# reinforcement-learning-kr/alpha_omok

Measured on AMD Instinct MI355X. Metric: self-play move-decisions/sec (9x9, 400 sims/move), higher is better.
Workload: dtype f32 (fp16x2-split MFMA operands, 3 products per multiply-add, f32 accumulate; inter-layer activations stored as two fp16 halves: ~22 significand bits)

## Files before the change

### alpha_omok_amd/csrc/net.hip

```cpp
#include <hip/hip_runtime.h>

#include <cmath>
#include <cstdio>
#include <cstdlib>
#include <cstring>
#include <map>
#include <type_traits>
#include <string>
#include <thread>
#include <vector>

#include "../../include/omok_hip.h"
#include "engine_types.hpp"
#include "net_device.hpp"
#include "net_common.hpp"
#include "net_trunk_f32.hpp"
#include "net_trunk_h16.hpp"
#include "net_layer_ksplit.hpp"
#include "net_board_h16.hpp"
#include "net_small.hpp"
#include "net_w16.hpp"


struct ao_net {
    int nb = 0, C = 0, planes = 0, B = 0, A = 0, device = 0;
    int nchq32 = 0;
    int nchq16 = 0;
    int CQ = 0;
    int mode = 0;
    int requested_mode = 0;
    int fp16_fallbacks = 0;
    bool forced_fp32 = false;
    int num_cu = 256;
    bool finalized = false;
    std::string err;
    std::map<std::string, std::vector<float>> params;
    std::vector<void*> allocs;
    std::vector<std::pair<void*, size_t>> pallocs;
    size_t pcursor = 0;
    std::vector<float*> conv_w, conv_sc, conv_sh;
    std::vector<uint4*> convh_wh, convh_wl;
    uint4 *step_w1h = nullptr, *step_w1l = nullptr;
    std::vector<float*> convh_sc;
    float* conv0_w16 = nullptr;
    float* conv0_w1 = nullptr;
    int nchq1 = 0;
    float *head_w3 = nullptr, *head_sc3 = nullptr, *head_sh3 = nullptr;
    float *wp_t = nullptr, *bp = nullptr, *w1_t = nullptr, *b1 = nullptr, *w2 = nullptr, *b2 = nullptr;
    int ws_boards = 0;
    float *act_x = nullptr, *act_t = nullptr, *hbuf = nullptr, *il_in = nullptr;
    float *tmp_p = nullptr, *tmp_v = nullptr;
    int* d_status = nullptr;
    bool attr_l[16][2] = {}, attr_done[16] = {}, lds_attr_done[16] = {}, attr_k[16] = {};
    int ksplit_min = 48, ksplit_max = 64, ksplit_max2 = 0;
    int rowk_min = 1, rowk_max = 47;
    bool attr_r[16] = {};
    int boardk_min = 64;
    bool attr_b[16] = {};
    long perboard_cells = 2592;
    int force_xt = 0, force_nch = 0;
    bool timing = false;
    bool timing_on = false;
    int timing_stride = 1;
    unsigned timing_tick = 0;
    static constexpr int kRing = 512;
    std::vector<hipEvent_t> ev0, ev1;
    int ring_head = 0, ring_count = 0;
    double ms_total = 0.0;
    int64_t launches = 0;
    int last_in_kind = 1;
    bool w16 = false;
    int products_req = 0;
    int trunk_fmt = -1;

    int fail(const std::string& m) { err = m; return 1; }
};

#define NET_HIP(n, call)                                                                      \
    do {                                                                                      \
        hipError_t st_ = (call);                                                              \
        if (st_ != hipSuccess)                                                                \
            return (n)->fail(std::string(#call) + ": " + hipGetErrorString(st_));             \
    } while (0)

static thread_local std::string g_net_create_error;

template <typename T>
static int net_alloc(ao_net* n, T** out, size_t count) {
    void* p = nullptr;
    hipError_t st = hipMalloc(&p, std::max<size_t>(count * sizeof(T), 16));
    if (st != hipSuccess) return n->fail(std::string("hipMalloc: ") + hipGetErrorString(st));
    n->allocs.push_back(p);
    *out = static_cast<T*>(p);
    return 0;
}

template <typename T>
static int param_alloc(ao_net* n, T** out, size_t count) {
    const size_t bytes = std::max<size_t>(count * sizeof(T), 16);
    if (n->pcursor < n->pallocs.size() && n->pallocs[n->pcursor].second == bytes) {
        *out = static_cast<T*>(n->pallocs[n->pcursor++].first);
        return 0;
    }
    void* p = nullptr;
    hipError_t st = hipMalloc(&p, bytes);
    if (st != hipSuccess) return n->fail(std::string("hipMalloc: ") + hipGetErrorString(st));
    if (n->pcursor < n->pallocs.size()) {
        (void)hipFree(n->pallocs[n->pcursor].first);
        n->pallocs[n->pcursor] = {p, bytes};
    } else {
        n->pallocs.push_back({p, bytes});
    }
    ++n->pcursor;
// ... 243 lines not shown
            switch (n->B) {
#define AO_CELLS_LAUNCH2(W, Q, NWV)                                                                           \
    hipLaunchKernelGGL((k_conv_cells<W, Q, NWV>), grid, block, 0, s, reinterpret_cast<const float4*>(in), w4, \
                       reinterpret_cast<const float4*>(n->conv_sc[layer]),                                   \
                       reinterpret_cast<const float4*>(n->conv_sh[layer]), reinterpret_cast<const float4*>(res), \
                       reinterpret_cast<float4*>(out), cqi, n->planes, res ? 1 : 0)
#define AO_CELLS_LAUNCH(W, Q)                                                                                 \
    do {                                                                                                      \
        if (nw == 9) AO_CELLS_LAUNCH2(W, Q, 9);                                                               \
        else AO_CELLS_LAUNCH2(W, Q, 3);                                                                       \
    } while (0)
#define AO_BW_CASE(W)                                                                                         \
    case W:                                                                                                   \
        switch (cqi >> 2) {                                                                                   \
            case 1: AO_CELLS_LAUNCH(W, 1); break;                                                             \
            case 2: AO_CELLS_LAUNCH(W, 2); break;                                                             \
            case 4: AO_CELLS_LAUNCH(W, 4); break;                                                             \
            case 6: AO_CELLS_LAUNCH(W, 6); break;                                                             \
            default: AO_CELLS_LAUNCH(W, 8); break;                                                            \
        }                                                                                                     \
        break;
                AO_BW_CASE(3) AO_BW_CASE(4) AO_BW_CASE(5) AO_BW_CASE(6) AO_BW_CASE(7) AO_BW_CASE(8) AO_BW_CASE(9)
                AO_BW_CASE(10) AO_BW_CASE(11) AO_BW_CASE(12) AO_BW_CASE(13) AO_BW_CASE(14) AO_BW_CASE(15)
#undef AO_BW_CASE
#undef AO_CELLS_LAUNCH
#undef AO_CELLS_LAUNCH2
            }
            if (timed) timer_end(n, idx, s);
        };
        if (parts & 1) conv(0, in_il, n->nchq1, nullptr, n->act_x);
        for (int i = 0; i < n->nb && (parts & 2); ++i) {
            conv(1 + 2 * i, n->act_x, n->CQ, nullptr, n->act_t);
            conv(2 + 2 * i, n->act_t, n->CQ, n->act_x, n->act_x);
        }
        const size_t lds1 = heads_lds_floats(n->A, n->planes) * sizeof(float);
        if (parts & 4)
            hipLaunchKernelGGL(k_heads_board, dim3(boards), dim3(1024), lds1, s, head_params(n),
                               reinterpret_cast<const float4*>(n->act_x), policy, value, n->A, n->planes);
        NET_HIP(n, hipGetLastError());
#ifdef AO_PROF
        if (getenv("AO_PROF_PRINT")) {
            unsigned long long h[8];
            hipStreamSynchronize(s);
            hipMemcpyFromSymbol(h, HIP_SYMBOL(ao_prof_heads), sizeof(h));
            unsigned long long cv[8];
            hipMemcpyFromSymbol(cv, HIP_SYMBOL(ao_prof_conv), sizeof(cv));
            fprintf(stderr, "AO_PROF k_conv_cells_h (last layer, block 0, wave 0) ticks: rows loaded + split + stored %llu, barrier + LDS reads + MFMAs %llu, reduction barrier %llu, reduce+epilogue+store %llu, total %llu\n",
                    cv[1] - cv[0], cv[2] - cv[1], cv[3] - cv[2], cv[4] - cv[3], cv[4] - cv[0]);
            fprintf(stderr, "AO_PROF k_heads_board ticks: w3 %llu, 1x1 conv %llu, reduce %llu, FC %llu, softmax+value %llu, tanh/store %llu, total %llu\n",
                    h[1] - h[0], h[2] - h[1], h[3] - h[2], h[4] - h[3], h[5] - h[4], h[6] - h[5], h[6] - h[0]);
        }
#endif
        return 0;
#ifdef AO_PROF
    } else if (group == 16 && mode == 5 && (layers_only(n) || !(n->B <= 9 && (groups >= 192 || getenv("AO_FORCE_RESIDENT"))))) {
#else
    } else if (group == 16 && mode == 5 && (layers_only(n) || !(n->B <= 9 && groups >= 192))) {
#endif
        int xt = n->B, nchh = 1;
        {
            double best = -1.0;
            const int xts[2] = {5, 4};
            for (int k = 0; k < (n->B <= 9 ? 1 : 2); ++k) {
                const int x = n->B <= 9 ? n->B : xts[k];
                const int ntile = (n->B + x - 1) / x;
                const int staged_cols = n->B <= 9 ? x : x + 2;
                for (int c = 1; c <= n->B; ++c) {
                    const long rounds = (static_cast<long>(groups) * c * ntile + n->num_cu - 1) / n->num_cu;
                    const int rows = (n->B + c - 1) / c;
                    const int staged_rows = rows + (c > 1 ? 2 : 0);
                    const double cost = rounds * (static_cast<double>(rows) * x + 0.25 * staged_rows * staged_cols + 2.0);
                    if (best < 0 || cost < best) { best = cost; nchh = c; xt = x; }
                }
            }
            if (n->force_xt > 0 && n->B > 9) xt = n->force_xt;
            if (n->force_nch > 0) nchh = n->force_nch;
        }
        const int nxt = (n->B + xt - 1) / xt;
        const int ks = (!layers_only(n) && n->B >= 4 && n->B <= 9 && groups >= n->ksplit_min) ? (groups <= n->ksplit_max ? 4 : groups <= n->ksplit_max2 ? 2 : 0) : 0;
        const bool rowk = !layers_only(n) && n->B >= 4 && n->B <= 9 && groups >= n->rowk_min && groups <= n->rowk_max;
        const bool ksplit = ks != 0 || rowk;
        auto layer_k = [&](int l) -> int {
            LayerHArgs a;
            a.src = static_cast<const void*>((l & 1) ? n->act_x : n->act_t);
            a.dst = reinterpret_cast<uint4*>(!(l & 1) ? n->act_x : n->act_t);
            a.layer.wh = n->convh_wh[l];
            a.layer.wl = n->convh_wl[l];
            a.layer.sc = reinterpret_cast<const float4*>(n->convh_sc[l]);
            a.layer.sh = reinterpret_cast<const float4*>(n->conv_sh[l]);
            a.layer.ovf = n->d_status;
            a.res = !(l & 1) ? 1 : 0;
            a.nch = groups;
            a.live = live; a.row_cap = row_cap;
            const dim3 grid(rowk ? (groups + 7) / 8 * 8 * 4 * n->B : (groups + 7) / 8 * 8 * ks), block(512);
            const int idx = n->timing ? timer_begin(n, s) : 0;
            if (two_products(n) && (rowk || ks == 4)) {
                if (rowk) NET_HIP(n, ao::launch_row16hk_w16(n->device, n->B, grid, s, a));
                else NET_HIP(n, ao::launch_layer16hk_w16(n->device, n->B, grid, s, a));
                if (n->timing) timer_end(n, idx, s);
                return 0;
            }
            if (rowk) {
                switch (n->B) {
#define AO_BW_CASE(W)                                                                                                  \
    case W: {                                                                                                          \
        constexpr size_t lds_ = static_cast<size_t>(W) * 8 * 1024;                                                     \
        if (!n->attr_r[W]) {                                                                                           \
            NET_HIP(n, hipFuncSetAttribute(reinterpret_cast<const void*>(&k_row16hk<W>),                               \
                                           hipFuncAttributeMaxDynamicSharedMemorySize, static_cast<int>(lds_)));       \
            n->attr_r[W] = true;                                                                                       \
        }                                                                                                              \
// ... 290 lines not shown
namespace ao {
void net_fp16_fallback_begin(ao_net* n) {
    ++n->fp16_fallbacks;
    n->mode = 2;
}
int net_fp16_fallback_end(ao_net* n) {
    n->forced_fp32 = n->fp16_fallbacks >= 3;
    if (!n->forced_fp32) n->mode = n->requested_mode;
    return n->forced_fp32 ? 1 : 0;
}
}

extern "C" {

const char* ao_net_last_error(const ao_net* n) { return n ? n->err.c_str() : g_net_create_error.c_str(); }

int ao_net_create(int n_block, int inplanes, int planes, int board, int device, ao_net** out) {
    if (!out) return 1;
    *out = nullptr;
    auto bad = [&](const char* m) { g_net_create_error = m; return 1; };
    if (n_block < 0 || n_block > 64) return bad("n_block out of range");
    if (inplanes < 1 || inplanes > 12) return bad("inplanes must be in 1..12");
    if (planes < 32 || planes > 512 || planes % 32) return bad("planes must be a multiple of 32 in 32 .. 512");
    if (board < 3 || board > ao::kMaxBoard) return bad("board must be in 3..15");
    int ndev = 0;
    if (hipGetDeviceCount(&ndev) != hipSuccess || ndev <= 0) return bad("no HIP device available");
    if (device < 0 || device >= ndev) return bad("device ordinal out of range");
    ao_net* n = new ao_net();
    n->nb = n_block; n->C = inplanes; n->planes = planes; n->B = board; n->A = board * board;
    n->device = device;
    n->nchq32 = (((inplanes + 3) / 4) + 1) & ~1;
    n->nchq16 = (((inplanes + 3) / 4) + 7) & ~7;
    n->nchq1 = (((inplanes + 3) / 4) + 3) & ~3;
    n->CQ = planes / 4;
    {
        hipDeviceProp_t prop;
        if (hipGetDeviceProperties(&prop, device) == hipSuccess && prop.multiProcessorCount > 0)
            n->num_cu = prop.multiProcessorCount;
    }
    if (const char* v = getenv("AO_KSPLIT")) {
        int lo = 0, hi = 0, hi2 = 0;
        if (sscanf(v, "%d,%d,%d", &lo, &hi, &hi2) == 3) { n->ksplit_min = lo > 0 ? lo : 1 << 30; n->ksplit_max = hi; n->ksplit_max2 = hi2; }
    }
    if (const char* v = getenv("AO_PERBOARD_CELLS")) n->perboard_cells = atol(v);
    if (const char* v = getenv("AO_BOARDK")) n->boardk_min = atoi(v);
    if (const char* v = getenv("AO_ROWK")) {
        int lo = 0, hi = -1;
        if (sscanf(v, "%d,%d", &lo, &hi) == 2) { n->rowk_min = lo; n->rowk_max = hi; }
    }
    if (const char* v = getenv("AO_TRUNK_FMT")) n->trunk_fmt = atoi(v) == 1 ? 1 : 0;
    if (n->trunk_fmt < 0) n->trunk_fmt = 0;
    if (const char* v = getenv("AO_XT")) n->force_xt = atoi(v) == 4 ? 4 : (atoi(v) == 5 ? 5 : 0);
    if (const char* v = getenv("AO_NCH")) n->force_nch = atoi(v) > 0 && atoi(v) <= board ? atoi(v) : 0;
    *out = n;
    return 0;
}

void ao_net_destroy(ao_net* n) {
    if (!n) return;
    hipSetDevice(n->device);
    hipDeviceSynchronize();
    for (void* p : n->allocs) hipFree(p);
    for (auto& pa : n->pallocs) hipFree(pa.first);
    for (auto e : n->ev0) hipEventDestroy(e);
    for (auto e : n->ev1) hipEventDestroy(e);
    delete n;
}

int ao_net_set_mode(ao_net* n, int mode) {
    if (mode < 0 || mode > 6)
        return n->fail("mode must be 0 (auto), 1 (layer kernels), 2 (group-resident trunk), 3 (per-board), 4 (row-chunked), 5 (split-fp16 trunk) "
                       "or 6 (split-fp16 per-layer kernels for every batch size)");
    if ((mode == 5 || mode == 6) && !h16_supported(n))
        return n->fail("modes 5 / 6 (split-fp16 MFMA trunk) need 128 planes and at least one ResBlock");
    n->mode = n->requested_mode = mode;
    n->forced_fp32 = false;
    return 0;
}


int ao_net_get_mode(const ao_net* n) { return n->mode; }

int ao_net_set_param(ao_net* n, const char* name, const float* data, int64_t numel) {
    if (!name || (!data && numel > 0) || numel < 0) return n->fail("bad argument");
    n->params[name] = std::vector<float>(data, data + numel);
    n->finalized = false;
    return 0;
}

static int get_param(ao_net* n, const std::string& name, size_t numel, const std::vector<float>** out) {
    auto it = n->params.find(name);
    if (it == n->params.end()) return n->fail("missing parameter " + name);
    if (it->second.size() != numel)
        return n->fail("parameter " + name + " has " + std::to_string(it->second.size()) + " elements, expected " +
                       std::to_string(numel));
    *out = &it->second;
    return 0;
}

static int fold_bn(ao_net* n, const std::string& prefix, int c, std::vector<float>* sc, std::vector<float>* sh) {
    const std::vector<float>*w, *b, *m, *v;
    if (get_param(n, prefix + ".weight", c, &w) || get_param(n, prefix + ".bias", c, &b) ||
        get_param(n, prefix + ".running_mean", c, &m) || get_param(n, prefix + ".running_var", c, &v))
        return 1;
    sc->resize(c); sh->resize(c);
    for (int i = 0; i < c; ++i) {
// ... 213 lines not shown
    NET_HIP(n, hipSetDevice(n->device));
    hipStream_t s = static_cast<hipStream_t>(stream);
    int32_t f = 0;
    NET_HIP(n, hipMemcpyAsync(&f, n->d_status, sizeof(int32_t), hipMemcpyDeviceToHost, s));
    NET_HIP(n, hipStreamSynchronize(s));
    if (clear && f) {
        NET_HIP(n, hipMemsetAsync(n->d_status, 0, sizeof(int32_t), s));
        NET_HIP(n, hipStreamSynchronize(s));
    }
    if (flags) *flags = f;
    return 0;
}

int ao_net_conv_timing(ao_net* n, int enable, double* ms_total, int64_t* launches) {
    NET_HIP(n, hipSetDevice(n->device));
    if (n->ev0.empty() && enable) {
        n->ev0.resize(ao_net::kRing);
        n->ev1.resize(ao_net::kRing);
        for (int i = 0; i < ao_net::kRing; ++i) {
            NET_HIP(n, hipEventCreate(&n->ev0[i]));
            NET_HIP(n, hipEventCreate(&n->ev1[i]));
        }
    }
    harvest(n, n->ring_count);
    if (ms_total) *ms_total = n->ms_total;
    if (launches) *launches = n->launches;
    n->ms_total = 0.0;
    n->launches = 0;
    n->timing_on = enable != 0;
    n->timing_stride = enable > 1 ? enable : 1;
    n->timing_tick = 0;
    n->timing = false;
    return 0;
}

static void dominant_name(const ao_net* n, int boards, int in_kind, std::string* nm_out, double* f_out) {
    int group = 32, nchq = 0;
    ao::net_plan(n, boards, &group, &nchq, nullptr);
    const int padded = (boards + group - 1) / group * group;
    const double conv = 2.0 * n->A * 9.0 * n->planes * n->planes * padded;
    const double conv1 = 2.0 * n->A * 9.0 * n->C * n->planes * padded;
    const int mode = ao::pick_mode_public(n, boards);
    const std::string bw = std::to_string(n->B);
    std::string nm;
    double f;
    if (group == 1) {
        nm = h16_supported(n) ? std::string(two_products(n) ? "k_conv_cells_h_w16<" : "k_conv_cells_h<") + bw + ", 8> (one 3x3 conv, per-board NHWC, board rows in LDS, split-fp16 MFMA 16x16x32, " +
                                    (two_products(n) ? "2 products: the conv weights are fp16 numbers)" : "3 products)")
                              : "k_conv_cells<" + bw + "> (one 3x3 conv, per-board NHWC, fp32 MFMA 16x16x4)";
        f = conv;
    } else if (group == 16 && mode == 4) {
        nm = "k_layer16<" + bw + "> (one 3x3 conv per launch, 16-board groups x row chunks, fp32 MFMA 16x16x4)";
        f = conv;
    } else if (group == 16 && mode == 5 && !layers_only(n) && n->B >= 4 && n->B <= 9 && (boards + 15) / 16 >= n->rowk_min &&
               (boards + 15) / 16 <= n->rowk_max) {
        nm = std::string(two_products(n) ? "k_row16hk_w16<" : "k_row16hk<") + bw + "> (one 3x3 conv per launch as split-fp16 MFMA 16x16x32 (" +
             (two_products(n) ? "2 products: the conv weights are fp16 numbers" : "3 products") + ", fp32 accumulate): one workgroup per "
             "16-board group x output row x cout pair, waves split the contraction by input block, partial tiles exchanged through LDS)";
        f = conv;
    } else if (group == 16 && mode == 5 && !layers_only(n) && n->B >= 4 && n->B <= 9 && (boards + 15) / 16 >= n->ksplit_min &&
               (boards + 15) / 16 <= std::max(n->ksplit_max, n->ksplit_max2)) {
        const bool four = (boards + 15) / 16 <= n->ksplit_max;
        const bool two = two_products(n) && four;
        nm = std::string(two ? "k_layer16hk_w16<" : "k_layer16hk<") + bw + (four ? ", 4" : ", 2") + "> (one 3x3 conv per launch as split-fp16 MFMA 16x16x32 (" +
             (two ? "2 products: the conv weights are fp16 numbers" : "3 products") + ", fp32 accumulate): "
             "a 16-board group split over " + (four ? "four workgroups by cout pairs" : "two workgroups by cout quads") +
             ", waves split the contraction by input block, partial tiles exchanged through LDS)";
        f = conv;
    } else if (group == 16 && mode == 5 && board_resident(n, boards)) {
        nm = std::string(two_products(n) ? "k_boardh_w16<" : "k_boardh<") + bw + (in_kind == 2 ? ", 2" : ", 1") + "> (" + (in_kind == 2 ? "conv1 + " : "") + std::to_string(2 * n->nb) +
             " 3x3 convs in one launch as split-fp16 MFMA 16x16x32 (" + (two_products(n) ? "2 products: the conv weights are fp16 numbers" : "3 products") + ", fp32 accumulate): "
             "a workgroup = one board resident in LDS through all layers, the row's cells as the MFMA N dimension, column shifts as DPP row shifts)";
        f = 2.0 * n->nb * 2.0 * n->A * 9.0 * n->planes * n->planes * boards + (in_kind == 2 ? 2.0 * n->A * 9.0 * n->C * n->planes * boards : 0.0);
    } else if (group == 16 && mode == 5 && (layers_only(n) || !(n->B <= 9 && (boards + 15) / 16 >= 192))) {
        nm = std::string(two_products(n) ? "k_layer16h_w16<" : "k_layer16h<") + bw + "> (one 3x3 conv per launch as split-fp16 MFMA 16x16x32 (" +
             (two_products(n) ? "2 products: the conv weights are fp16 numbers" : "3 products") + ", fp32 accumulate), "
             "16-board groups x row chunks x column tiles)";
        f = conv;
    } else if (group == 16 && mode == 5) {
        const bool two = two_products(n) && n->trunk_fmt != 1;
        nm = std::string(in_kind == 2 ? "k_trunk16hb" : "k_trunk16h") + (two ? "_w16<" : "<") + bw + ", 4, " + std::to_string(n->trunk_fmt) + "> (conv1 + " +
             std::to_string(2 * n->nb) + " 3x3 convs as split-fp16 MFMA 16x16x32 (" + (two ? "2 products: the conv weights are fp16 numbers" : "3 products") + ", fp32 accumulate) + heads, one resident "
             "launch; activations between layers as " + (n->trunk_fmt == 1 ? "fp16 high half + one low byte" : "two fp16 halves") + ")";
        f = conv1 + 2.0 * n->nb * conv;
    } else if (group == 16) {
        nm = "k_trunk16<" + bw + "> (conv1 + " + std::to_string(2 * n->nb) + " 3x3 convs, one launch, fp32 MFMA 16x16x4)";
        f = conv1 + 2.0 * n->nb * conv;
    } else {
        nm = "k_conv3x3<" + bw + "> (one 3x3 " + std::to_string(n->planes) + "->" + std::to_string(n->planes) +
             " conv, fp32 MFMA 32x32x2)";
        f = conv;
    }
    *nm_out = nm;
    *f_out = f;
}

static void copy_name(const std::string& nm, char* name, int name_cap) {
    if (name && name_cap > 0) {
        std::strncpy(name, nm.c_str(), static_cast<size_t>(name_cap) - 1);
        name[name_cap - 1] = 0;
    }
}

int ao_net_products(ao_net* n, int32_t request, int32_t* in_force, int32_t* weights_fp16) {
    if (request != -1 && request != 0 && request != 3) return n->fail("ao_net_products: request must be -1 (query), 0 (automatic) or 3");
    if (request != -1) n->products_req = request;
    if (in_force) *in_force = two_products(n) ? 2 : 3;
    if (weights_fp16) *weights_fp16 = n->w16 ? 1 : 0;
    return 0;
}

int ao_net_dominant_kernel(ao_net* n, int boards, char* name, int name_cap, double* flop_per_launch) {
    std::string nm;
    double f = 0.0;
    dominant_name(n, boards, n->last_in_kind, &nm, &f);
    copy_name(nm, name, name_cap);
    if (flop_per_launch) *flop_per_launch = f;
    return 0;
}

int ao_net_plan_kernel(int n_block, int inplanes, int planes, int board, int trunk_mode, int boards, int in_kind,
                       char* name, int name_cap, double* flop_per_launch) {
    if (n_block < 0 || inplanes < 1 || planes < 32 || planes % 32 || board < 3 || board > ao::kMaxBoard || boards < 1 ||
        trunk_mode < 0 || trunk_mode > 6)
        return 1;
    ao_net n;
    n.nb = n_block; n.C = inplanes; n.planes = planes; n.B = board; n.A = board * board;
// ... 17 lines not shown
```

### alpha_omok_amd/csrc/net_trunk_h16.hpp

```cpp
#pragma once

namespace ao {

struct TrunkHLayer {
    const uint4* wh;
    const uint4* wl;
    const float4* sc;
    const float4* sh;
    int* ovf;
};

struct TrunkHArgs {
    const float4* in0;
    uint4* bufA;
    uint4* bufB;
    int nlayers;
    int CQ, COUT;
    const float *w3, *sc3, *sh3, *wp_t, *bp, *w1_t, *b1, *w2, *b2;
    float* policy;
    float* value;
    const unsigned* live;
    unsigned row_cap;
    TrunkHLayer layers[kMaxTrunkLayers];
};

typedef unsigned int u32x2 __attribute__((ext_vector_type(2)));
__device__ __forceinline__ half8 buf_ld_h8(__amdgpu_buffer_rsrc_t r, int voff, int soff) {
    return __builtin_bit_cast(half8, __builtin_amdgcn_raw_buffer_load_b128(r, voff, soff, 0));
}
#ifndef AO_AUX_RES
#define AO_AUX_RES 0
#endif
#ifndef AO_AUX_ST
#define AO_AUX_ST 0
#endif
#ifndef AO_AUX_STAGE
#define AO_AUX_STAGE 0
#endif
__device__ __forceinline__ half4 buf_ld_h4(__amdgpu_buffer_rsrc_t r, int voff, int soff) {
    return __builtin_bit_cast(half4, __builtin_amdgcn_raw_buffer_load_b64(r, voff, soff, AO_AUX_RES));
}
__device__ __forceinline__ void buf_st_h4(half4 v, __amdgpu_buffer_rsrc_t r, int voff, int soff) {
    __builtin_amdgcn_raw_buffer_store_b64(__builtin_bit_cast(u32x2, v), r, voff, soff, AO_AUX_ST);
}

#ifdef AO_PROF
static __device__ unsigned long long ao_prof[8 * 12];
#define AO_T(x) const unsigned long long x = __builtin_amdgcn_s_memtime()
#define AO_ACC(k, t0, t1) prof[k] += (t1) - (t0)
#else
#define AO_T(x)
#define AO_ACC(k, t0, t1)
#endif
// ... 9 lines not shown
}
__device__ __forceinline__ uint4 ao_ko_fragment(unsigned seed, bool low) {
    unsigned wd[4];
#pragma unroll
    for (int k = 0; k < 4; ++k) {
        unsigned out = 0;
#pragma unroll
        for (int h = 0; h < 2; ++h) {
            const unsigned r = ao_ko_hash(seed * 8u + k * 2u + h);
            const unsigned e = (low ? 4u : 15u) - ((r >> 10) & 7u);
            const unsigned v = (r & 0x80000000u) ? 0u : ((e << 10) | (r & 0x3ffu));
            out |= v << (16 * h);
        }
        wd[k] = out;
    }
    return make_uint4(wd[0], wd[1], wd[2], wd[3]);
}
#if AO_KO != 0 && !defined(AO_PROF) && !defined(AO_WRONG_RESULTS_OK)
#error "AO_KO builds compute wrong results on purpose: timing only, build them with -DAO_PROF"
#endif
#ifndef AO_SPLIT_BARRIER
#define AO_SPLIT_BARRIER 0
#endif
#ifndef AO_CONV1_SPLIT
#define AO_CONV1_SPLIT 0
#endif
__device__ __forceinline__ void row_arrive(unsigned* cnt, int lane) {
    asm volatile("s_waitcnt vmcnt(0) lgkmcnt(0)" ::: "memory");
    if (lane == 0) __hip_atomic_fetch_add(cnt, 1u, __ATOMIC_RELAXED, __HIP_MEMORY_SCOPE_WORKGROUP);
}
__device__ __forceinline__ void row_wait(unsigned* cnt, unsigned target) {
    for (;;) {
        const unsigned v = __hip_atomic_load(cnt, __ATOMIC_RELAXED, __HIP_MEMORY_SCOPE_WORKGROUP);
        if (__builtin_amdgcn_readfirstlane(v) >= target) break;
        __builtin_amdgcn_s_sleep(1);
    }
    asm volatile("" ::: "memory");
}

__host__ __device__ constexpr int kPlaneRow(int bw) { return bw * bw <= 128 ? 128 : 256; }
__host__ __device__ constexpr unsigned kPairBytes(int fmt) { return fmt == 1 ? 1536u : 2048u; }

constexpr float kLo8Scale = 0x1p-112f;
__device__ __forceinline__ float lo8_scaled(unsigned h, unsigned l) { return __uint_as_float(((h << 8) | l) << 5); }
__device__ __forceinline__ unsigned lo8_word(float vs) {
    const unsigned u = __float_as_uint(vs);
    return (u + 15u + ((u >> 5) & 1u)) >> 5;
}

template <int BW, int NC32, int NCI, int KIND, int FMT = 0, bool W16 = false>
struct TrunkHLayerFn {
static __device__ __forceinline__ void run(const void* src, uint4* dst, const TrunkHLayer& L, const bool RES, uint4* s_x,
                                           int tile, int lane, unsigned long long* prof, const bool flip,
                                           unsigned* s_cnt, const unsigned rows_before) {
    constexpr bool FIRST = KIND != 0;
    constexpr bool BITS = KIND == 2;
    auto py = [&](int y) { return flip ? BW - 1 - y : y; };
    constexpr int A = BW * BW;
    constexpr int NT = NC32 * 2;
    constexpr int NSP = 2;
    constexpr int NFR = BW * NCI * NSP;
    constexpr int NB = NCI * 3;
    constexpr int NPR = 3;
    constexpr int PAIR = static_cast<int>(kPairBytes(FMT));
    constexpr int NPAIR = BW * NCI;
    const int kq = lane >> 4, b = lane & 15;
    const int lane16 = lane * 16;
    const int out_voff = (((tile & 1) * 2 + (kq >> 1)) * 16 + b) * 16 + (kq & 1) * 8;
    float4 sc = L.sc[tile * 4 + kq], sh = L.sh[tile * 4 + kq];
    if (FMT == 1) {
        sc.x *= kLo8Scale; sc.y *= kLo8Scale; sc.z *= kLo8Scale; sc.w *= kLo8Scale;
        sh.x *= kLo8Scale; sh.y *= kLo8Scale; sh.z *= kLo8Scale; sh.w *= kLo8Scale;
    }
    const __amdgpu_buffer_rsrc_t rs_wh = make_rsrc(L.wh, 9u * NCI * NT * 1024u);
    const __amdgpu_buffer_rsrc_t rs_wl = make_rsrc(L.wl, 9u * NCI * NT * 1024u);
    const __amdgpu_buffer_rsrc_t rs_src =
        make_rsrc(src, BITS ? 16u * kPlaneRow(BW) : FIRST ? static_cast<unsigned>(A) * 8u * 16u * 16u : static_cast<unsigned>(A) * NCI * kPairBytes(FMT));
    const __amdgpu_buffer_rsrc_t rs_dst = make_rsrc(dst, static_cast<unsigned>(A) * NC32 * kPairBytes(FMT));
    half8 wA[2][3], wB[2][3], wres[2][FIRST ? 9 : 1];
    auto load_w = [&](int slab, half8 (&W)[2][3]) {
        if (FIRST) return;
        if (AO_KO == 1 && slab > 2) return;
        const int c = (slab / 3) % NCI, dy = slab % 3;
#pragma unroll
        for (int dx = 0; dx < 3; ++dx) {
            const int ub = ((((flip ? 2 - dy : dy) * 3 + dx) * NCI + c) * NT + tile) * 1024;
            W[0][dx] = buf_ld_h8(rs_wh, lane16, ub);
            if (!W16) W[1][dx] = buf_ld_h8(rs_wl, lane16, ub);
        }
    };
    if (FIRST) {
#pragma unroll
        for (int t = 0; t < 9; ++t) {
            wres[0][t] = buf_ld_h8(rs_wh, lane16, (t * NT + tile) * 1024);
            if (!W16) wres[1][t] = buf_ld_h8(rs_wl, lane16, (t * NT + tile) * 1024);
        }
    }
    auto load_planes = [&](int cell, int split) -> half8 {
        if (BITS) {
            const unsigned bits = __builtin_amdgcn_raw_buffer_load_b8(rs_src, b * kPlaneRow(BW) + cell, 0, 0);
            half8 h;
#pragma unroll
            for (int k = 0; k < 8; ++k)
                h[k] = (kq == 0 && split == 0 && ((bits >> k) & 1u)) ? static_cast<_Float16>(1.0f) : static_cast<_Float16>(0.0f);
            return h;
        }
        const int o = ((cell * 8 + 2 * kq) * 16 + b) * 16;
        const u32x4 q0 = __builtin_amdgcn_raw_buffer_load_b128(rs_src, o, 0, 0);
        const u32x4 q1 = __builtin_amdgcn_raw_buffer_load_b128(rs_src, o + 256, 0, 0);
        half8 h;
#pragma unroll
        for (int k = 0; k < 4; ++k) {
            const float v0 = __uint_as_float(q0[k]), v1 = __uint_as_float(q1[k]);
            const _Float16 h0 = static_cast<_Float16>(v0), h1 = static_cast<_Float16>(v1);
            h[k] = split ? static_cast<_Float16>(v0 - static_cast<float>(h0)) : h0;
            h[4 + k] = split ? static_cast<_Float16>(v1 - static_cast<float>(h1)) : h1;
        }
        return h;
    };
    float peak = 0.f;
    unsigned pbits[BITS ? (NFR + NT - 1) / NT : 1] = {};
    f32x4 acc[3][BW];
#pragma unroll
    for (int r = 0; r < 3; ++r)
#pragma unroll
        for (int i = 0; i < BW; ++i) acc[r][i] = f32x4{0.f, 0.f, 0.f, 0.f};
    auto epilogue = [&](int yo) {
        constexpr int HB = (BW + 1) / 2;
#pragma unroll
        for (int i0 = 0; i0 < BW; i0 += HB) {
            half4 rh[HB], rl[HB];
            unsigned rb[HB];
            if (RES) {
#pragma unroll
                for (int k = 0; k < HB; ++k) {
                    const int i = i0 + k < BW ? i0 + k : BW - 1;
                    const int ob = ((py(yo) * BW + i) * NC32 + (tile >> 1)) * PAIR;
                    rh[k] = buf_ld_h4(rs_dst, out_voff, ob);
                    if (FMT == 1) {
                        rb[k] = __builtin_amdgcn_raw_buffer_load_b32(rs_dst, out_voff >> 1, ob + 1024, AO_AUX_RES);
                    } else if (AO_KO == 10 || AO_KO == 12) {
                        const unsigned u = __builtin_amdgcn_raw_buffer_load_b32(rs_dst, out_voff >> 1, ob + 1024, AO_AUX_RES);
                        rl[k] = __builtin_bit_cast(half4, u32x2{u, u});
                    } else {
                        rl[k] = buf_ld_h4(rs_dst, out_voff, ob + 1024);
                    }
                }
            }
#pragma unroll
            for (int k = 0; k < HB; ++k) {
                const int i = i0 + k;
                if (i >= BW) continue;
                const f32x4 c = acc[0][i];
                float f[4] = {fmaf(c[0], sc.x, sh.x), fmaf(c[1], sc.y, sh.y), fmaf(c[2], sc.z, sh.z), fmaf(c[3], sc.w, sh.w)};
                const int ob = ((py(yo) * BW + i) * NC32 + (tile >> 1)) * PAIR;
                if (RES) {
                    if (FMT == 1) {
                        const u32x2 hb = __builtin_bit_cast(u32x2, rh[k]);
#pragma unroll
                        for (int r = 0; r < 4; ++r)
                            f[r] += lo8_scaled((hb[r >> 1] >> (16 * (r & 1))) & 0xffffu, (rb[k] >> (8 * r)) & 0xffu);
                    } else {
#pragma unroll
                        for (int r = 0; r < 4; ++r) f[r] += static_cast<float>(rh[k][r]) + static_cast<float>(rl[k][r]);
                    }
                }
                peak = fmaxf(fmaxf(peak, fmaxf(f[0], f[1])), fmaxf(f[2], f[3]));
                if (FMT == 1) {
                    unsigned t[4];
#pragma unroll
                    for (int r = 0; r < 4; ++r)
                        t[r] = lo8_word(f[r] >= 0x1p-126f ? fminf(f[r], 65504.f * kLo8Scale) : 0.f);
                    const u32x2 hw = {(t[0] >> 8) | ((t[1] >> 8) << 16), (t[2] >> 8) | ((t[3] >> 8) << 16)};
                    const unsigned lw = (t[0] & 0xffu) | ((t[1] & 0xffu) << 8) | ((t[2] & 0xffu) << 16) | (t[3] << 24);
                    __builtin_amdgcn_raw_buffer_store_b64(hw, rs_dst, out_voff, ob, AO_AUX_ST);
                    __builtin_amdgcn_raw_buffer_store_b32(lw, rs_dst, out_voff >> 1, ob + 1024, AO_AUX_ST);
                    continue;
                }
                half4 hh, hl;
#pragma unroll
                for (int r = 0; r < 4; ++r) {
                    const float v = fminf(fmaxf(f[r], 0.f), 65504.f);
                    hh[r] = static_cast<_Float16>(v);
                    hl[r] = static_cast<_Float16>(v - static_cast<float>(hh[r]));
                }
                buf_st_h4(hh, rs_dst, out_voff, ob);
                if (AO_KO == 10 || AO_KO == 12) __builtin_amdgcn_raw_buffer_store_b32(__builtin_bit_cast(u32x2, hl)[0], rs_dst, out_voff >> 1, ob + 1024, AO_AUX_ST);
                else
                buf_st_h4(hl, rs_dst, out_voff, ob + 1024);
            }
        }
    };
    auto stage_pairs = [&](int y, uint4* xb, int k0, int k1) {
#pragma unroll
        for (int k = k0; k < k1; ++k) {
            const int p = tile + NT * k;
            if (p < NPAIR) {
                const int so = (py(y) * NPAIR + p) * PAIR;
                __builtin_amdgcn_raw_ptr_buffer_load_lds(rs_src, (__attribute__((address_space(3))) void*)(xb + (2 * p) * 64), 16, lane16,
                                                         so, 0, AO_AUX_STAGE);
                if (lane < 32)
                    __builtin_amdgcn_raw_ptr_buffer_load_lds(rs_src, (__attribute__((address_space(3))) void*)(xb + (2 * p + 1) * 64), 16,
                                                             lane16, so + 1024, 0, AO_AUX_STAGE);
            }
        }
    };
    auto expand_pairs = [&](uint4* xb, int k0, int k1) {
        typedef _Float16 half2v __attribute__((ext_vector_type(2)));
        const half2v k18 = {static_cast<_Float16>(0x1p-18f), static_cast<_Float16>(0x1p-18f)};
        const half2v m8 = {static_cast<_Float16>(-0x1p-8f), static_cast<_Float16>(-0x1p-8f)};
#pragma unroll
        for (int k = k0; k < k1; ++k) {
            const int p = tile + NT * k;
            if (p < NPAIR) {
                const uint4 hv = xb[(2 * p) * 64 + lane];
                const u32x2 lv = reinterpret_cast<const u32x2*>(xb + (2 * p + 1) * 64)[lane];
                const unsigned hw[4] = {hv.x, hv.y, hv.z, hv.w};
                unsigned ow[4];
#pragma unroll
                for (int j = 0; j < 4; ++j) {
                    const unsigned y = __builtin_amdgcn_perm(0x64646464u, lv[j >> 1], (j & 1) ? 0x04030402u : 0x04010400u);
                    const half2v c = __builtin_elementwise_fma(__builtin_bit_cast(half2v, y), k18, m8);
                    const half2v sc2 = __builtin_bit_cast(half2v, hw[j] & 0x7c007c00u);
                    ow[j] = __builtin_bit_cast(unsigned, c * sc2);
                }
                xb[(2 * p + 1) * 64 + lane] = make_uint4(ow[0], ow[1], ow[2], ow[3]);
            }
        }
    };

    AO_T(t_a);
    __syncthreads();
    AO_T(t_a1);
    if (FIRST) {
#pragma unroll
        for (int k = 0; k < (NFR + NT - 1) / NT; ++k) {
            const int f = tile + NT * k;
            if (f < NFR) s_x[f * 64 + lane] = __builtin_bit_cast(uint4, load_planes(f >> 1, f & 1));
        }
    } else if (FMT == 1) {
        stage_pairs(0, s_x, 0, (NPAIR + NT - 1) / NT);
    } else if (!(AO_KO == 13 || AO_KO == 15)) {
#pragma unroll
        for (int k = 0; k < (NFR + NT - 1) / NT; ++k) {
            const int f = tile + NT * k;
            if (f < NFR && !(AO_KO == 10 && (f & 1) && lane >= 32))
                __builtin_amdgcn_raw_ptr_buffer_load_lds(rs_src, (__attribute__((address_space(3))) void*)(s_x + f * 64), 16,
                                                         (AO_KO == 12 && (f & 1) && lane >= 32) ? lane16 - 512 : lane16,
                                                         (py(0) * NFR + f) * 1024, 0, AO_AUX_STAGE);
        }
    }
    AO_T(t_a2);
    load_w(0, wA);
    asm volatile("s_waitcnt vmcnt(0) lgkmcnt(0)" ::: "memory");
    if (FMT == 1 && !FIRST) {
        expand_pairs(s_x, 0, (NPAIR + NT - 1) / NT);
        asm volatile("s_waitcnt lgkmcnt(0)" ::: "memory");
    }
    AO_T(t_a3);
    __syncthreads();
    AO_T(t_b);
    AO_ACC(0, t_a, t_b);
    AO_ACC(8, t_a, t_a1);
    AO_ACC(9, t_a1, t_a2);
    AO_ACC(10, t_a2, t_a3);
    AO_ACC(11, t_a3, t_b);

    for (int yi = 0; yi < BW; ++yi) {
        AO_T(t_r0);
        const uint4* xs = s_x + static_cast<size_t>(yi & 1) * NFR * 64;
        uint4* xn = s_x + static_cast<size_t>((yi + 1) & 1) * NFR * 64;
        const int yn = yi + 1 < BW ? yi + 1 : yi;
#pragma unroll
        for (int slab = 0; slab < NB; ++slab) {
            const int c = slab / 3, dy = slab % 3;
            half8 (&w)[2][3] = (slab & 1) ? wB : wA;
            half8 (&wn)[2][3] = (slab & 1) ? wA : wB;
            load_w(slab + 1, wn);
            if (dy == 1 && !AO_KO_NOSTAGE && FMT == 1 && !FIRST) {
                constexpr int K2 = (NPAIR / NT + NCI - 1) / (NCI > 1 ? NCI - 1 : 1);
                if (c > 0 && AO_KO != 11) expand_pairs(xn, (c - 1) * K2, c * K2);
                if (c + 1 < NCI) stage_pairs(yn, xn, c * K2, (c + 1) * K2);
            } else if (BITS && !AO_KO_NOSTAGE && AO_CONV1_SPLIT) {
                constexpr int KF = (NFR + NT - 1) / NT;
#pragma unroll
                for (int k = 0; k < KF; ++k) {
                    const int f = tile + NT * k;
                    if (f < NFR) {
                        if (dy == 0 && !(f & 1))
                            pbits[k] = __builtin_amdgcn_raw_buffer_load_b8(rs_src, b * kPlaneRow(BW) + yn * BW + (f >> 1), 0, 0);
                        if (dy == 2) {
                            half8 h;
#pragma unroll
                            for (int q = 0; q < 8; ++q)
                                h[q] = (kq == 0 && !(f & 1) && ((pbits[k] >> q) & 1u)) ? static_cast<_Float16>(1.0f) : static_cast<_Float16>(0.0f);
                            xn[f * 64 + lane] = __builtin_bit_cast(uint4, h);
                        }
                    }
                }
            } else if (dy == 1 && (!AO_KO_NOSTAGE || FIRST)) {
#pragma unroll
                for (int k = 0; k < (NFR / NT + NCI) / NCI; ++k) {
                    const int f = tile + NT * (c * ((NFR / NT + NCI) / NCI) + k);
                    if (f < NFR) {
                        if (FIRST) xn[f * 64 + lane] = __builtin_bit_cast(uint4, load_planes(yn * BW + (f >> 1), f & 1));
                        else if (!(AO_KO == 10 && (f & 1) && lane >= 32))
                            __builtin_amdgcn_raw_ptr_buffer_load_lds(rs_src, (__attribute__((address_space(3))) void*)(xn + f * 64),
                                                                     16, (AO_KO == 12 && (f & 1) && lane >= 32) ? lane16 - 512 : lane16,
                                                                     (py(yn) * NFR + f) * 1024, 0, AO_AUX_STAGE);
                    }
                }
            }
            const int yo = yi + 1 - dy;
            if (yo >= 0 && yo < BW) {
                half8 xh = __builtin_bit_cast(half8, xs[((0 * NCI + c) * NSP + 0) * 64 + lane]);
                half8 xl = __builtin_bit_cast(half8, xs[((0 * NCI + c) * NSP + 1) * 64 + lane]);
#pragma unroll
                for (int xi = 0; xi < BW; ++xi) {
                    half8 nh = xh, nl = xl;
                    if (xi + 1 < BW && AO_KO != 2) {
                        nh = __builtin_bit_cast(half8, xs[(((xi + 1) * NCI + c) * NSP + 0) * 64 + lane]);
                        nl = __builtin_bit_cast(half8, xs[(((xi + 1) * NCI + c) * NSP + 1) * 64 + lane]);
                    }
#pragma unroll
                    for (int pr = 0; pr < NPR; ++pr) {
                        if (BITS && pr == 2) continue;
                        if (W16 && pr == 1) continue;
#pragma unroll
                        for (int dx = 0; dx < 3; ++dx) {
                            const int i = xi - dx + 1;
                            if (i < 0 || i >= BW) continue;
                            const half8 wv = FIRST ? wres[pr == 1 ? 1 : 0][FIRST ? dy * 3 + dx : 0] : w[pr == 1 ? 1 : 0][dx];
                            acc[2 - dy][i] = __builtin_amdgcn_mfma_f32_16x16x32_f16(wv, pr == 2 ? xl : xh, acc[2 - dy][i], 0, 0, 0);
                        }
                    }
                    xh = nh;
                    xl = nl;
                    __builtin_amdgcn_sched_barrier(0);
                }
            }
            __builtin_amdgcn_sched_barrier(0);
        }
        AO_T(t_r1);
#if AO_SPLIT_BARRIER
        row_arrive(s_cnt, lane);
#endif
        if (yi >= 1 && (!AO_KO_NOEPI || (AO_KO == 4 && yi == 1))) epilogue(yi - 1);
        else if (yi >= 1 && (AO_KO == 14 || AO_KO == 15)) {
#pragma unroll
            for (int i = 0; i < BW; ++i) asm volatile("" ::"v"(acc[0][i]));
        }
#pragma unroll
        for (int i = 0; i < BW; ++i) {
            acc[0][i] = acc[1][i];
            acc[1][i] = acc[2][i];
            acc[2][i] = f32x4{0.f, 0.f, 0.f, 0.f};
        }
        AO_T(t_r2);
#if AO_SPLIT_BARRIER
        if (yi + 1 < BW && AO_KO != 9) row_wait(s_cnt, static_cast<unsigned>(NT) * (rows_before + static_cast<unsigned>(yi) + 1u));
#else
        if (AO_KO == 9) asm volatile("s_waitcnt vmcnt(0) lgkmcnt(0)" ::: "memory");
        else asm volatile("s_waitcnt vmcnt(0) lgkmcnt(0)\n\ts_barrier" ::: "memory");
#endif
        AO_T(t_r3);
        AO_ACC(1, t_r0, t_r1);
        AO_ACC(2, t_r1, t_r2);
        AO_ACC(3, t_r2, t_r3);
    }
    AO_T(t_c);
    if (!AO_KO_NOEPI || FIRST) epilogue(BW - 1);
    if (peak > (FMT == 1 ? 65504.f * kLo8Scale : 65504.f)) atomicOr(L.ovf, 1);
    asm volatile("s_waitcnt vmcnt(0)" ::: "memory");
    __syncthreads();
    __builtin_amdgcn_fence(__ATOMIC_ACQUIRE, "workgroup");
    AO_T(t_d);
    AO_ACC(4, t_c, t_d);
}
};

template <int BW, int XT, int NC32, int NCI, int KIND, bool W16 = false>
__device__ __forceinline__ void trunk_h_layer_tile(const void* src, uint4* dst, const TrunkHLayer& L, const bool RES,
                                                   uint4* s_x, int tile, int lane, int x0, int yb, int ye) {
    constexpr bool FIRST = KIND != 0;
    constexpr bool BITS = KIND == 2;
    constexpr int A = BW * BW;
    constexpr bool HALO = XT < BW;
    constexpr int NX = HALO ? XT + 2 : XT;
    constexpr int NT = NC32 * 2;
    constexpr int NSP = 2;
    constexpr int NFR = NX * NCI * NSP;
    constexpr int NB = NCI * 3;
    constexpr int NPR = 3;
    const int kq = lane >> 4, b = lane & 15;
    const int lane16 = lane * 16;
    const int out_voff = (((tile & 1) * 2 + (kq >> 1)) * 16 + b) * 16 + (kq & 1) * 8;
    const float4 sc = L.sc[tile * 4 + kq], sh = L.sh[tile * 4 + kq];
    const __amdgpu_buffer_rsrc_t rs_wh = make_rsrc(L.wh, 9u * NCI * NT * 1024u);
    const __amdgpu_buffer_rsrc_t rs_wl = make_rsrc(L.wl, 9u * NCI * NT * 1024u);
    const __amdgpu_buffer_rsrc_t rs_src =
        make_rsrc(src, BITS ? 16u * kPlaneRow(BW) : FIRST ? static_cast<unsigned>(A) * 8u * 16u * 16u : static_cast<unsigned>(A) * NCI * 2u * 1024u);
    const __amdgpu_buffer_rsrc_t rs_dst = make_rsrc(dst, static_cast<unsigned>(A) * NC32 * 2u * 1024u);
    half8 wA[2][3], wB[2][3], wres[2][FIRST ? 9 : 1];
    auto load_w = [&](int slab, half8 (&W)[2][3]) {
        if (FIRST) return;
        const int c = (slab / 3) % NCI, dy = slab % 3;
#pragma unroll
        for (int dx = 0; dx < 3; ++dx) {
            const int ub = (((dy * 3 + dx) * NCI + c) * NT + tile) * 1024;
            W[0][dx] = buf_ld_h8(rs_wh, lane16, ub);
            if (!W16) W[1][dx] = buf_ld_h8(rs_wl, lane16, ub);
        }
    };
    if (FIRST) {
#pragma unroll
        for (int t = 0; t < 9; ++t) {
            wres[0][t] = buf_ld_h8(rs_wh, lane16, (t * NT + tile) * 1024);
            if (!W16) wres[1][t] = buf_ld_h8(rs_wl, lane16, (t * NT + tile) * 1024);
        }
    }
    auto load_planes = [&](int cell, int split) -> half8 {
        if (BITS) {
            const unsigned bits = __builtin_amdgcn_raw_buffer_load_b8(rs_src, b * kPlaneRow(BW) + cell, 0, 0);
            half8 h;
// ... 154 lines not shown
    constexpr int NXT = (BW + XT - 1) / XT;
    extern __shared__ __attribute__((aligned(16))) uint4 s_x[];
    const int xt = blockIdx.x % NXT;
    const int rest = blockIdx.x / NXT;
    const int grp = rest / a.nch, ch = rest - grp * a.nch;
    if (grp >= live_groups16(a.live, a.row_cap, grp + 1)) return;
    const int base = BW / a.nch, extra = BW % a.nch;
    const int yb = ch * base + (ch < extra ? ch : extra);
    const int ye = yb + base + (ch < extra ? 1 : 0);
    const int lane = threadIdx.x & 63;
    const int tile = __builtin_amdgcn_readfirstlane(static_cast<int>(threadIdx.x) >> 6);
    uint4* dst = a.dst + static_cast<size_t>(grp) * A * NC32 * 2 * 64;
    if (KIND == 2) {
        trunk_h_layer_tile<BW, XT, NC32, 1, 2, W16>(static_cast<const uint8_t*>(a.src) + static_cast<size_t>(grp) * 16 * kPlaneRow(BW), dst,
                                               a.layer, false, s_x, tile, lane, xt * XT, yb, ye);
    } else if (KIND == 1) {
        trunk_h_layer_tile<BW, XT, NC32, 1, 1, W16>(static_cast<const float4*>(a.src) + static_cast<size_t>(grp) * A * 8 * 16, dst, a.layer,
                                               false, s_x, tile, lane, xt * XT, yb, ye);
    } else {
        trunk_h_layer_tile<BW, XT, NC32, NC32, 0, W16>(static_cast<const uint4*>(a.src) + static_cast<size_t>(grp) * A * NC32 * 2 * 64, dst,
                                                      a.layer, a.res != 0, s_x, tile, lane, xt * XT, yb, ye);
    }
}

template <int BW, int XT, int NC32, int KIND>
__global__ __launch_bounds__(NC32 * 2 * 64, 1) void k_layer16h(LayerHArgs a) {
    layer16h_body<BW, XT, NC32, KIND, false>(a);
}
template <int BW, int XT, int NC32, int KIND>
__global__ __launch_bounds__(NC32 * 2 * 64, 1) void k_layer16h_w16(LayerHArgs a) {
    layer16h_body<BW, XT, NC32, KIND, true>(a);
}

template <int BW, int NC32, int INK, int FMT, bool W16 = false>
__device__ __forceinline__ void trunk16h_body(const TrunkHArgs& a) {
    static_assert(FMT == 0 || AO_SPLIT_BARRIER == 0, "the split row barrier is implemented for the 4-byte format only");
    constexpr int A = BW * BW;
    extern __shared__ __attribute__((aligned(16))) uint4 s_x[];
    const int grp = blockIdx.x;
    if (grp >= live_groups16(a.live, a.row_cap, grp + 1)) return;
    const int lane = threadIdx.x & 63;
    const int tile = __builtin_amdgcn_readfirstlane(static_cast<int>(threadIdx.x) >> 6);
    const size_t gq = static_cast<size_t>(AO_KO == 5 ? grp % 64 : AO_KO == 6 ? grp % 128 : grp) * A * NC32 * (kPairBytes(FMT) / 16);
    uint4* bufA = a.bufA + gq;
    uint4* bufB = a.bufB + gq;
    unsigned long long prof[12] = {0, 0, 0, 0, 0, 0, 0, 0, 0, 0, 0, 0};
    unsigned long long* pp = prof;
    unsigned* s_cnt = reinterpret_cast<unsigned*>(s_x + static_cast<size_t>(2) * BW * NC32 * 2 * 64);
    if (threadIdx.x == 0) *s_cnt = 0u;
    const bool ko_fill = AO_KO == 13 || AO_KO == 15;
    AO_T(t0);
    if (INK == 2)
        TrunkHLayerFn<BW, NC32, 1, 2, FMT, W16>::run(reinterpret_cast<const uint8_t*>(a.in0) + static_cast<size_t>(grp) * 16 * kPlaneRow(BW), bufA,
                                      a.layers[0], false, s_x, tile, lane, pp, false, s_cnt, 0u);
    else
        TrunkHLayerFn<BW, NC32, 1, 1, FMT, W16>::run(a.in0 + static_cast<size_t>(grp) * A * 8 * 16, bufA, a.layers[0], false, s_x, tile, lane, pp, false,
                                      s_cnt, 0u);
    AO_T(t1);
    if (ko_fill) {
        __syncthreads();
        for (int f = tile; f < 2 * BW * NC32 * 2; f += NC32 * 2) s_x[f * 64 + lane] = ao_ko_fragment((grp * 4u * BW * NC32 + f) * 64u + lane, f & 1);
        __syncthreads();
    }
#ifdef AO_PROF
    for (int k = 0; k < 12; ++k) prof[k] = 0;
#endif
    for (int l = 1; l < a.nlayers; ++l) {
        const bool second = (l & 1) == 0;
        TrunkHLayerFn<BW, NC32, NC32, 0, FMT, W16>::run(second ? bufB : bufA, second ? bufA : bufB, a.layers[l], second, s_x, tile, lane, pp,
                                             (l & 1) != 0, s_cnt, static_cast<unsigned>(l) * BW);
    }
    AO_T(t2);
    if (AO_KO != 8) trunk_heads<BW, FMT == 1 ? 2 : 1>(a, reinterpret_cast<const float4*>(a.bufA), static_cast<size_t>(grp) * A, grp);
#ifdef AO_PROF
    AO_T(t3);
    prof[5] = t3 - t2;
    prof[6] = t1 - t0;
    prof[7] = t3 - t0;
    if (grp == 5 && lane == 0)
        for (int k = 0; k < 12; ++k) ao_prof[tile * 12 + k] = prof[k];
#endif
}

template <int BW, int NC32, int FMT>
__global__ __launch_bounds__(NC32 * 2 * 64, 1) void k_trunk16h(TrunkHArgs a) {
    trunk16h_body<BW, NC32, 1, FMT>(a);
}
template <int BW, int NC32, int FMT>
__global__ __launch_bounds__(NC32 * 2 * 64, 1) void k_trunk16hb(TrunkHArgs a) {
    trunk16h_body<BW, NC32, 2, FMT>(a);
}
template <int BW, int NC32, int FMT>
__global__ __launch_bounds__(NC32 * 2 * 64, 1) void k_trunk16h_w16(TrunkHArgs a) {
    trunk16h_body<BW, NC32, 1, FMT, true>(a);
}
template <int BW, int NC32, int FMT>
__global__ __launch_bounds__(NC32 * 2 * 64, 1) void k_trunk16hb_w16(TrunkHArgs a) {
    trunk16h_body<BW, NC32, 2, FMT, true>(a);
}

}
```

Baseline: 6685.

## Hand off last two output rows through LDS to next resident trunk layer

In the board-resident split-fp16 trunk kernel, each layer's epilogue for its final two output rows now writes the fp16 hi/lo halves straight into the LDS row buffers the next layer reads first. The next layer skips its initial global load of those rows, along with the vmcnt wait and barrier. A parity offset tracks which LDS buffer holds which row across layers, and the global store is skipped when the output is not needed for a residual. The aim is to cut the global round-trip and synchronisation at every layer boundary. A separate change moves the AO_FORCE_RESIDENT env override out of the profile-only build into a normal config flag.

New measurement: 6829, median of 6. 1.02x the previous value.

```diff
diff --git a/alpha_omok_amd/csrc/net.hip b/alpha_omok_amd/csrc/net.hip
--- a/alpha_omok_amd/csrc/net.hip
+++ b/alpha_omok_amd/csrc/net.hip
@@ -59,6 +59,7 @@
     bool attr_b[16] = {};
     long perboard_cells = 2592;
     int force_xt = 0, force_nch = 0;
+    bool force_resident = false;
     bool timing = false;
     bool timing_on = false;
     int timing_stride = 1;
@@ -408,11 +409,7 @@
         }
 #endif
         return 0;
-#ifdef AO_PROF
-    } else if (group == 16 && mode == 5 && (layers_only(n) || !(n->B <= 9 && (groups >= 192 || getenv("AO_FORCE_RESIDENT"))))) {
-#else
-    } else if (group == 16 && mode == 5 && (layers_only(n) || !(n->B <= 9 && groups >= 192))) {
-#endif
+    } else if (group == 16 && mode == 5 && (layers_only(n) || !(n->B <= 9 && (groups >= 192 || n->force_resident)))) {
         int xt = n->B, nchh = 1;
         {
             double best = -1.0;
@@ -809,6 +806,7 @@
     if (n->trunk_fmt < 0) n->trunk_fmt = 0;
     if (const char* v = getenv("AO_XT")) n->force_xt = atoi(v) == 4 ? 4 : (atoi(v) == 5 ? 5 : 0);
     if (const char* v = getenv("AO_NCH")) n->force_nch = atoi(v) > 0 && atoi(v) <= board ? atoi(v) : 0;
+    if (const char* v = getenv("AO_FORCE_RESIDENT")) n->force_resident = atoi(v) != 0;
     *out = n;
     return 0;
 }
@@ -1128,13 +1126,13 @@
     } else if (group == 16 && mode == 4) {
         nm = "k_layer16<" + bw + "> (one 3x3 conv per launch, 16-board groups x row chunks, fp32 MFMA 16x16x4)";
         f = conv;
-    } else if (group == 16 && mode == 5 && !layers_only(n) && n->B >= 4 && n->B <= 9 && (boards + 15) / 16 >= n->rowk_min &&
+    } else if (group == 16 && mode == 5 && !layers_only(n) && !n->force_resident && n->B >= 4 && n->B <= 9 && (boards + 15) / 16 >= n->rowk_min &&
                (boards + 15) / 16 <= n->rowk_max) {
         nm = std::string(two_products(n) ? "k_row16hk_w16<" : "k_row16hk<") + bw + "> (one 3x3 conv per launch as split-fp16 MFMA 16x16x32 (" +
              (two_products(n) ? "2 products: the conv weights are fp16 numbers" : "3 products") + ", fp32 accumulate): one workgroup per "
              "16-board group x output row x cout pair, waves split the contraction by input block, partial tiles exchanged through LDS)";
         f = conv;
-    } else if (group == 16 && mode == 5 && !layers_only(n) && n->B >= 4 && n->B <= 9 && (boards + 15) / 16 >= n->ksplit_min &&
+    } else if (group == 16 && mode == 5 && !layers_only(n) && !n->force_resident && n->B >= 4 && n->B <= 9 && (boards + 15) / 16 >= n->ksplit_min &&
                (boards + 15) / 16 <= std::max(n->ksplit_max, n->ksplit_max2)) {
         const bool four = (boards + 15) / 16 <= n->ksplit_max;
         const bool two = two_products(n) && four;
@@ -1148,7 +1146,7 @@
              " 3x3 convs in one launch as split-fp16 MFMA 16x16x32 (" + (two_products(n) ? "2 products: the conv weights are fp16 numbers" : "3 products") + ", fp32 accumulate): "
              "a workgroup = one board resident in LDS through all layers, the row's cells as the MFMA N dimension, column shifts as DPP row shifts)";
         f = 2.0 * n->nb * 2.0 * n->A * 9.0 * n->planes * n->planes * boards + (in_kind == 2 ? 2.0 * n->A * 9.0 * n->C * n->planes * boards : 0.0);
-    } else if (group == 16 && mode == 5 && (layers_only(n) || !(n->B <= 9 && (boards + 15) / 16 >= 192))) {
+    } else if (group == 16 && mode == 5 && (layers_only(n) || !(n->B <= 9 && ((boards + 15) / 16 >= 192 || n->force_resident)))) {
         nm = std::string(two_products(n) ? "k_layer16h_w16<" : "k_layer16h<") + bw + "> (one 3x3 conv per launch as split-fp16 MFMA 16x16x32 (" +
              (two_products(n) ? "2 products: the conv weights are fp16 numbers" : "3 products") + ", fp32 accumulate), "
              "16-board groups x row chunks x column tiles)";
diff --git a/alpha_omok_amd/csrc/net_trunk_h16.hpp b/alpha_omok_amd/csrc/net_trunk_h16.hpp
--- a/alpha_omok_amd/csrc/net_trunk_h16.hpp
+++ b/alpha_omok_amd/csrc/net_trunk_h16.hpp
@@ -1,4 +1,6 @@
 #pragma once
+
+#include <type_traits>
 
 namespace ao {
 
@@ -114,14 +116,18 @@
 struct TrunkHLayerFn {
 static __device__ __forceinline__ void run(const void* src, uint4* dst, const TrunkHLayer& L, const bool RES, uint4* s_x,
                                            int tile, int lane, unsigned long long* prof, const bool flip,
-                                           unsigned* s_cnt, const unsigned rows_before) {
+                                           unsigned* s_cnt, const unsigned rows_before, const bool hand_next, const int par) {
     constexpr bool FIRST = KIND != 0;
     constexpr bool BITS = KIND == 2;
+    constexpr bool HAND = FMT == 0 && AO_KO == 0;
+    constexpr bool HANDED = HAND && !FIRST;
+    static_assert(!HAND || NC32 >= 2, "conv1's hand-off assumes that its own row buffers lie inside the next layer's buffer 0");
     auto py = [&](int y) { return flip ? BW - 1 - y : y; };
     constexpr int A = BW * BW;
     constexpr int NT = NC32 * 2;
     constexpr int NSP = 2;
     constexpr int NFR = BW * NCI * NSP;
+    constexpr int NFRO = BW * NC32 * NSP;
     constexpr int NB = NCI * 3;
     constexpr int NPR = 3;
     constexpr int PAIR = static_cast<int>(kPairBytes(FMT));
@@ -187,7 +193,8 @@
     for (int r = 0; r < 3; ++r)
 #pragma unroll
         for (int i = 0; i < BW; ++i) acc[r][i] = f32x4{0.f, 0.f, 0.f, 0.f};
-    auto epilogue = [&](int yo) {
+    auto epilogue = [&](int yo, auto ho, uint4* hx) {
+        constexpr bool HO = decltype(ho)::value;
         constexpr int HB = (BW + 1) / 2;
 #pragma unroll
         for (int i0 = 0; i0 < BW; i0 += HB) {
@@ -246,6 +253,12 @@
                     hh[r] = static_cast<_Float16>(v);
                     hl[r] = static_cast<_Float16>(v - static_cast<float>(hh[r]));
                 }
+                if (HO) {
+                    u32x2* hp = reinterpret_cast<u32x2*>(reinterpret_cast<char*>(hx) + (i * NC32 + (tile >> 1)) * 2048 + out_voff);
+                    hp[0] = __builtin_bit_cast(u32x2, hh);
+                    hp[128] = __builtin_bit_cast(u32x2, hl);
+                    if (!RES && !FIRST) continue;
+                }
                 buf_st_h4(hh, rs_dst, out_voff, ob);
                 if (AO_KO == 10 || AO_KO == 12) __builtin_amdgcn_raw_buffer_store_b32(__builtin_bit_cast(u32x2, hl)[0], rs_dst, out_voff >> 1, ob + 1024, AO_AUX_ST);
                 else
@@ -291,6 +304,11 @@
         }
     };
 
+    const int po = (BW & 1) ? 0 : par;
+    uint4* const hand2 = s_x + static_cast<size_t>(FIRST ? 1 : (BW + po) & 1) * NFRO * 64;
+    uint4* const hand1 = s_x + static_cast<size_t>(FIRST ? 0 : (BW - 1 + po) & 1) * NFRO * 64;
+    constexpr std::integral_constant<bool, true> kHand{};
+    constexpr std::integral_constant<bool, false> kStore{};
     AO_T(t_a);
     __syncthreads();
     AO_T(t_a1);
@@ -300,6 +318,7 @@
             const int f = tile + NT * k;
             if (f < NFR) s_x[f * 64 + lane] = __builtin_bit_cast(uint4, load_planes(f >> 1, f & 1));
         }
+    } else if (HANDED) {
     } else if (FMT == 1) {
         stage_pairs(0, s_x, 0, (NPAIR + NT - 1) / NT);
     } else if (!(AO_KO == 13 || AO_KO == 15)) {
@@ -314,13 +333,13 @@
     }
     AO_T(t_a2);
     load_w(0, wA);
-    asm volatile("s_waitcnt vmcnt(0) lgkmcnt(0)" ::: "memory");
+    if (!HANDED) asm volatile("s_waitcnt vmcnt(0) lgkmcnt(0)" ::: "memory");
     if (FMT == 1 && !FIRST) {
         expand_pairs(s_x, 0, (NPAIR + NT - 1) / NT);
         asm volatile("s_waitcnt lgkmcnt(0)" ::: "memory");
     }
     AO_T(t_a3);
-    __syncthreads();
+    if (!HANDED) __syncthreads();
     AO_T(t_b);
     AO_ACC(0, t_a, t_b);
     AO_ACC(8, t_a, t_a1);
@@ -330,16 +349,18 @@
 
     for (int yi = 0; yi < BW; ++yi) {
         AO_T(t_r0);
-        const uint4* xs = s_x + static_cast<size_t>(yi & 1) * NFR * 64;
-        uint4* xn = s_x + static_cast<size_t>((yi + 1) & 1) * NFR * 64;
-        const int yn = yi + 1 < BW ? yi + 1 : yi;
+        const uint4* xs = s_x + static_cast<size_t>((yi + po) & 1) * NFR * 64;
+        uint4* xn = s_x + static_cast<size_t>((yi + 1 + po) & 1) * NFR * 64;
+        const int yn = yi + 1;
+        const bool stage_next = yn < BW && !(HANDED && yi == 0);
 #pragma unroll
         for (int slab = 0; slab < NB; ++slab) {
             const int c = slab / 3, dy = slab % 3;
             half8 (&w)[2][3] = (slab & 1) ? wB : wA;
             half8 (&wn)[2][3] = (slab & 1) ? wA : wB;
             load_w(slab + 1, wn);
-            if (dy == 1 && !AO_KO_NOSTAGE && FMT == 1 && !FIRST) {
+            if (!stage_next) {
+            } else if (dy == 1 && !AO_KO_NOSTAGE && FMT == 1 && !FIRST) {
                 constexpr int K2 = (NPAIR / NT + NCI - 1) / (NCI > 1 ? NCI - 1 : 1);
                 if (c > 0 && AO_KO != 11) expand_pairs(xn, (c - 1) * K2, c * K2);
                 if (c + 1 < NCI) stage_pairs(yn, xn, c * K2, (c + 1) * K2);
@@ -407,7 +428,10 @@
 #if AO_SPLIT_BARRIER
         row_arrive(s_cnt, lane);
 #endif
-        if (yi >= 1 && (!AO_KO_NOEPI || (AO_KO == 4 && yi == 1))) epilogue(yi - 1);
+        if (yi >= 1 && (!AO_KO_NOEPI || (AO_KO == 4 && yi == 1))) {
+            if (HAND && hand_next && yi == BW - 1) epilogue(yi - 1, kHand, hand2);
+            else epilogue(yi - 1, kStore, nullptr);
+        }
         else if (yi >= 1 && (AO_KO == 14 || AO_KO == 15)) {
 #pragma unroll
             for (int i = 0; i < BW; ++i) asm volatile("" ::"v"(acc[0][i]));
@@ -420,7 +444,7 @@
         }
         AO_T(t_r2);
 #if AO_SPLIT_BARRIER
-        if (yi + 1 < BW && AO_KO != 9) row_wait(s_cnt, static_cast<unsigned>(NT) * (rows_before + static_cast<unsigned>(yi) + 1u));
+        if ((yi + 1 < BW || (HAND && hand_next)) && AO_KO != 9) row_wait(s_cnt, static_cast<unsigned>(NT) * (rows_before + static_cast<unsigned>(yi) + 1u));
 #else
         if (AO_KO == 9) asm volatile("s_waitcnt vmcnt(0) lgkmcnt(0)" ::: "memory");
         else asm volatile("s_waitcnt vmcnt(0) lgkmcnt(0)\n\ts_barrier" ::: "memory");
@@ -431,7 +455,10 @@
         AO_ACC(3, t_r2, t_r3);
     }
     AO_T(t_c);
-    if (!AO_KO_NOEPI || FIRST) epilogue(BW - 1);
+    if (!AO_KO_NOEPI || FIRST) {
+        if (HAND && hand_next) epilogue(BW - 1, kHand, hand1);
+        else epilogue(BW - 1, kStore, nullptr);
+    }
     if (peak > (FMT == 1 ? 65504.f * kLo8Scale : 65504.f)) atomicOr(L.ovf, 1);
     asm volatile("s_waitcnt vmcnt(0)" ::: "memory");
     __syncthreads();
@@ -692,10 +719,10 @@
     AO_T(t0);
     if (INK == 2)
         TrunkHLayerFn<BW, NC32, 1, 2, FMT, W16>::run(reinterpret_cast<const uint8_t*>(a.in0) + static_cast<size_t>(grp) * 16 * kPlaneRow(BW), bufA,
-                                      a.layers[0], false, s_x, tile, lane, pp, false, s_cnt, 0u);
+                                      a.layers[0], false, s_x, tile, lane, pp, false, s_cnt, 0u, a.nlayers > 1, 0);
     else
         TrunkHLayerFn<BW, NC32, 1, 1, FMT, W16>::run(a.in0 + static_cast<size_t>(grp) * A * 8 * 16, bufA, a.layers[0], false, s_x, tile, lane, pp, false,
-                                      s_cnt, 0u);
+                                      s_cnt, 0u, a.nlayers > 1, 0);
     AO_T(t1);
     if (ko_fill) {
         __syncthreads();
@@ -705,10 +732,12 @@
 #ifdef AO_PROF
     for (int k = 0; k < 12; ++k) prof[k] = 0;
 #endif
+    int par = 0;
     for (int l = 1; l < a.nlayers; ++l) {
         const bool second = (l & 1) == 0;
         TrunkHLayerFn<BW, NC32, NC32, 0, FMT, W16>::run(second ? bufB : bufA, second ? bufA : bufB, a.layers[l], second, s_x, tile, lane, pp,
-                                             (l & 1) != 0, s_cnt, static_cast<unsigned>(l) * BW);
+                                             (l & 1) != 0, s_cnt, static_cast<unsigned>(l) * BW, l + 1 < a.nlayers, par);
+        par = (par + BW - 1) & 1;
     }
     AO_T(t2);
     if (AO_KO != 8) trunk_heads<BW, FMT == 1 ? 2 : 1>(a, reinterpret_cast<const float4*>(a.bufA), static_cast<size_t>(grp) * A, grp);
```
